# david-macmahon/BLDistributedDataProducts.jl

Measured on AMD Instinct MI355X. Metric: filterbank GB/s reduced (node) + % HBM roofline, 8-bank 0000 band, higher is better.
Workload: dtype f32

## Files before the change

bldistributeddataproducts.jl_amd/csrc/bslz4.hip:

```cpp
#include <algorithm>
#include <cstring>
#include <vector>

#include "bldp_impl.h"

namespace {

inline uint32_t be32(const uint8_t *p) {
  return (uint32_t)p[0] << 24 | (uint32_t)p[1] << 16 | (uint32_t)p[2] << 8 | p[3];
}
inline uint64_t be64(const uint8_t *p) { return (uint64_t)be32(p) << 32 | be32(p + 4); }

__host__ __device__ inline uint64_t transpose8(uint64_t x) {
  uint64_t t;
  t = (x ^ (x >> 7)) & 0x00AA00AA00AA00AAull;
  x = x ^ t ^ (t << 7);
  t = (x ^ (x >> 14)) & 0x0000CCCC0000CCCCull;
  x = x ^ t ^ (t << 14);
  t = (x ^ (x >> 28)) & 0x00000000F0F0F0F0ull;
  x = x ^ t ^ (t << 28);
  return x;
}

int64_t lz4_block_host(const uint8_t *src, size_t slen, uint8_t *dst, size_t dcap) {
  size_t ip = 0, op = 0;
  while (ip < slen) {
    const uint8_t token = src[ip++];
    size_t lit = token >> 4;
    if (lit == 15) {
      uint8_t b;
      do {
        if (ip >= slen) return -1;
        b = src[ip++];
        lit += b;
      } while (b == 255);
    }
    if (ip + lit > slen || op + lit > dcap) return -1;
    memcpy(dst + op, src + ip, lit);
    ip += lit;
    op += lit;
    if (ip >= slen) break;
    if (ip + 2 > slen) return -1;
    const size_t off = (size_t)src[ip] | (size_t)src[ip + 1] << 8;
    ip += 2;
    size_t ml = token & 15;
    if (ml == 15) {
      uint8_t b;
      do {
        if (ip >= slen) return -1;
        b = src[ip++];
        ml += b;
      } while (b == 255);
    }
    ml += 4;
    if (off == 0 || off > op || op + ml > dcap) return -1;
    for (size_t i = 0; i < ml; ++i) dst[op + i] = dst[op - off + i];
    op += ml;
  }
  return (int64_t)op;
}

void bitunshuffle_host(const uint8_t *planes, uint8_t *out, size_t n, size_t es) {
  const size_t rowb = n / 8;
  for (size_t g = 0; g < rowb; ++g)
    for (size_t j = 0; j < es; ++j) {
      uint64_t x = 0;
      for (int k = 0; k < 8; ++k) x |= (uint64_t)planes[(j * 8 + k) * rowb + g] << (8 * k);
      x = transpose8(x);
      for (int t = 0; t < 8; ++t) out[(8 * g + t) * es + j] = (uint8_t)(x >> (8 * t));
    }
}

struct Task {
  uint64_t src;
  uint64_t dst;
  uint32_t clen;
  uint32_t nelem;
};
constexpr uint32_t RAW = 0xFFFFFFFFu;

struct ChunkDesc {
  uint64_t src, len, dst;
  uint64_t n, block;
  uint32_t nfull, last, tail;
  uint32_t task0;
};

int describe_chunk(const uint8_t *c, uint64_t len, uint64_t src, uint64_t dst, int es,
                   ChunkDesc *d) {
  if (len < 12) return bldp::set_error(BLDP_EINVAL, "bslz4: chunk shorter than its header");
  const uint64_t nb = be64(c);
  const uint32_t bb = be32(c + 8);
  if (nb % es || bb % es || bb == 0 || (bb / es) % 8 || bb > (1u << 24))
    return bldp::set_error(BLDP_EINVAL, "bslz4: bad header (bytes %llu, block %u, elem %d)",
                           (unsigned long long)nb, bb, es);
  d->src = src;
  d->len = len;
  d->dst = dst;
  d->n = nb / es;
  d->block = bb / es;
  d->nfull = (uint32_t)(d->n / d->block);
  uint64_t last = d->n % d->block;
  d->last = (uint32_t)(last - last % 8);
  d->tail = (uint32_t)(d->n - (uint64_t)d->nfull * d->block - d->last);
  return BLDP_OK;
}

inline uint32_t ntasks(const ChunkDesc &d) {
  return d.nfull + (d.last ? 1 : 0) + (d.tail ? 1 : 0);
}

__host__ __device__ inline uint32_t lz4_bound(uint32_t n) { return n + n / 255 + 16; }

__device__ inline uint32_t be32_dev(const uint8_t *p) {
  return (uint32_t)p[0] << 24 | (uint32_t)p[1] << 16 | (uint32_t)p[2] << 8 | p[3];
}

__global__ __launch_bounds__(64) void k_bslz4_plan(const uint8_t *__restrict__ comp,
                                                   const ChunkDesc *__restrict__ chunks,
                                                   int nchunk, int es, uint32_t cap,
                                                   Task *__restrict__ tasks, int *err) {
  const int k = blockIdx.x * 64 + threadIdx.x;
  if (k >= nchunk) return;
  const ChunkDesc d = chunks[k];
  uint64_t pos = d.src + 12, e = 0;
  const uint64_t end = d.src + d.len;
  const uint32_t nblk = d.nfull + (d.last ? 1 : 0);
  for (uint32_t b = 0; b < nblk; ++b) {
    const uint32_t ne = b < d.nfull ? (uint32_t)d.block : d.last;
    if (pos + 4 > end) { atomicOr(err, 2); return; }
    const uint32_t cl = be32_dev(comp + pos);
    if (cl > cap || pos + 4 + cl > end) { atomicOr(err, 2); return; }
    tasks[d.task0 + b] = Task{pos + 4, d.dst + e * es, cl, ne};
    pos += 4 + cl;
    e += ne;
  }
  if (pos + (uint64_t)d.tail * es != end) { atomicOr(err, 4); return; }
  if (d.tail) tasks[d.task0 + nblk] = Task{pos, d.dst + e * es, RAW, d.tail};
}

int plan_chunk(const uint8_t *c, uint64_t len, uint64_t src0, uint64_t dst0, int es,
               std::vector<Task> &tasks, uint64_t *out_bytes, uint32_t *max_block) {
  if (len < 12) return bldp::set_error(BLDP_EINVAL, "bslz4: chunk shorter than its header");
  const uint64_t nb = be64(c);
  const uint32_t bb = be32(c + 8);
  if (nb % es || bb % es || bb == 0 || (bb / es) % 8)
    return bldp::set_error(BLDP_EINVAL, "bslz4: bad header (bytes %llu, block %u, elem %d)",
                           (unsigned long long)nb, bb, es);
  const uint64_t n = nb / es, block = bb / es;
  uint64_t pos = 12, e = 0;
  const uint64_t nfull = n / block;
  uint64_t last = n % block;
  last -= last % 8;
  for (uint64_t k = 0; k < nfull + (last ? 1 : 0); ++k) {
    const uint64_t ne = k < nfull ? block : last;
    if (pos + 4 > len) return bldp::set_error(BLDP_EINVAL, "bslz4: truncated block header");
    const uint32_t cl = be32(c + pos);
    if (cl == RAW || pos + 4 + cl > len)
      return bldp::set_error(BLDP_EINVAL, "bslz4: block %llu overruns the chunk",
                             (unsigned long long)k);
    tasks.push_back(Task{src0 + pos + 4, dst0 + e * es, cl, (uint32_t)ne});
    *max_block = std::max<uint32_t>(*max_block, std::max<uint32_t>(cl, (uint32_t)(ne * es)));
    pos += 4 + cl;
    e += ne;
  }
  const uint64_t tail = n - e;
  if (pos + tail * es != len)
    return bldp::set_error(BLDP_EINVAL, "bslz4: %llu trailing bytes, expected %llu",
                           (unsigned long long)(len - pos), (unsigned long long)(tail * es));
  if (tail) tasks.push_back(Task{src0 + pos, dst0 + e * es, RAW, (uint32_t)tail});
  *out_bytes = nb;
  return BLDP_OK;
}

__global__ __launch_bounds__(64) void k_bslz4(const uint8_t *__restrict__ comp,
                                              const Task *__restrict__ tasks, int ntask,
                                              uint8_t *__restrict__ out, int es, uint32_t cap,
                                              int *err) {
  extern __shared__ uint8_t lds[];
  const int lane = threadIdx.x;
  if (*err & 6) return;
  const Task t = tasks[blockIdx.x];
  if (t.clen == RAW) {
    for (uint32_t i = lane; i < t.nelem * (uint32_t)es; i += 64) out[t.dst + i] = comp[t.src + i];
    return;
  }
  uint8_t *in = lds, *dec = lds + cap;
  const uint32_t clen = t.clen, nbytes = t.nelem * (uint32_t)es;
  if (clen > cap) {
    if (lane == 0) atomicOr(err, 1);
    return;
  }
  for (uint32_t i = lane; i < clen; i += 64) in[i] = comp[t.src + i];
  __syncthreads();
  uint32_t ip = 0, op = 0;
  bool bad = false;
  while (ip < clen) {
    const uint32_t token = in[ip++];
    uint32_t lit = token >> 4;
    if (lit == 15) {
      uint32_t b;
      do {
        if (ip >= clen) { bad = true; break; }
        b = in[ip++];
        lit += b;
      } while (b == 255);
      if (bad) break;
    }
    if (ip + lit > clen || op + lit > nbytes) { bad = true; break; }
    for (uint32_t i = lane; i < lit; i += 64) dec[op + i] = in[ip + i];
    ip += lit;
    op += lit;
    if (ip >= clen) break;
    if (ip + 2 > clen) { bad = true; break; }
    const uint32_t off = (uint32_t)in[ip] | (uint32_t)in[ip + 1] << 8;
    ip += 2;
    uint32_t ml = token & 15;
    if (ml == 15) {
      uint32_t b;
      do {
        if (ip >= clen) { bad = true; break; }
        b = in[ip++];
        ml += b;
      } while (b == 255);
      if (bad) break;
    }
    ml += 4;
    if (off == 0 || off > op || op + ml > nbytes) { bad = true; break; }
    __syncthreads();
    const uint32_t step = off < 64 ? off : 64;
    for (uint32_t r = 0; r < ml; r += step) {
      const uint32_t i = r + lane;
      if (lane < step && i < ml) dec[op + i] = dec[op - off + i];
      __syncthreads();
    }
    op += ml;
  }
  if (bad || op != nbytes) {
    if (lane == 0) atomicOr(err, 1);
    return;
  }
  __syncthreads();
  const uint32_t rowb = t.nelem / 8;
  if (es == 4) {
    for (uint32_t g = lane; g < rowb; g += 64) {
      uint32_t w[8] = {0, 0, 0, 0, 0, 0, 0, 0};
#pragma unroll
      for (int j = 0; j < 4; ++j) {
        uint64_t x = 0;
#pragma unroll
        for (int k = 0; k < 8; ++k) x |= (uint64_t)dec[(j * 8 + k) * rowb + g] << (8 * k);
        x = transpose8(x);
#pragma unroll
        for (int q = 0; q < 8; ++q) w[q] |= (uint32_t)((x >> (8 * q)) & 0xFF) << (8 * j);
      }
      uint32_t *o = reinterpret_cast<uint32_t *>(out + t.dst) + 8 * g;
#pragma unroll
      for (int q = 0; q < 8; ++q) o[q] = w[q];
    }
  } else {
    for (uint32_t g = lane; g < rowb; g += 64)
      for (int j = 0; j < es; ++j) {
        uint64_t x = 0;
        for (int k = 0; k < 8; ++k) x |= (uint64_t)dec[(j * 8 + k) * rowb + g] << (8 * k);
        x = transpose8(x);
        for (int q = 0; q < 8; ++q) out[t.dst + (8 * g + q) * es + j] = (uint8_t)(x >> (8 * q));
      }
  }
}

}

extern "C" {

BLDP_API int bldp_bslz4_info(const void *chunk, size_t nbytes, uint64_t *uncompressed_bytes,
                             uint32_t *block_bytes) {
  if (!chunk || nbytes < 12 || !uncompressed_bytes || !block_bytes)
    return bldp::set_error(BLDP_EINVAL, "bslz4: null pointer or short chunk");
  *uncompressed_bytes = be64((const uint8_t *)chunk);
  *block_bytes = be32((const uint8_t *)chunk + 8);
  return BLDP_OK;
}

BLDP_API int bldp_bslz4_decode_host(const void *chunk, size_t nbytes, int elem_size, void *out,
                                    size_t out_bytes) {
  if (!chunk || (!out && out_bytes) || elem_size <= 0)
    return bldp::set_error(BLDP_EINVAL, "bslz4: bad argument");
  std::vector<Task> tasks;
  uint64_t total = 0;
  uint32_t maxb = 0;
  int rc = plan_chunk((const uint8_t *)chunk, nbytes, 0, 0, elem_size, tasks, &total, &maxb);
  if (rc) return rc;
  if (total != out_bytes)
    return bldp::set_error(BLDP_EINVAL, "bslz4: chunk holds %llu bytes, output has %zu",
                           (unsigned long long)total, out_bytes);
  const uint8_t *c = (const uint8_t *)chunk;
  uint8_t *o = (uint8_t *)out;
  std::vector<uint8_t> dec(maxb);
  for (const Task &t : tasks) {
    const size_t nb = (size_t)t.nelem * elem_size;
    if (t.clen == RAW) {
      memcpy(o + t.dst, c + t.src, nb);
      continue;
    }
    if (lz4_block_host(c + t.src, t.clen, dec.data(), nb) != (int64_t)nb)
      return bldp::set_error(BLDP_EINVAL, "bslz4: corrupt LZ4 block at byte %llu",
                             (unsigned long long)t.src);
    bitunshuffle_host(dec.data(), o + t.dst, t.nelem, elem_size);
  }
  return BLDP_OK;
}

static int decode_launch(int nchunk, const uint8_t *comp_host, const uint8_t *comp_dev,
                         const uint64_t *chunk_off, const uint64_t *chunk_len, int elem_size,
                         uint8_t *out_dev, const uint64_t *out_off, const uint64_t *out_len,
                         int *derr_user, hipStream_t s, int **derr_used,
                         bldp::ScratchLease &lease, uint64_t host_base = 0) {
  if (nchunk < 0 || (nchunk && (!comp_host || !comp_dev || !chunk_off || !chunk_len ||
                                !out_dev || !out_off || !out_len)) ||
      elem_size <= 0 || elem_size > 64)
    return bldp::set_error(BLDP_EINVAL, "bslz4: bad argument");
  if (elem_size == 4 && ((uintptr_t)out_dev & 3))
    return bldp::set_error(BLDP_EINVAL, "bslz4: output must be 4-byte aligned");
  std::vector<ChunkDesc> descs(nchunk);
  uint64_t ntask = 0;
  uint32_t maxbb = 0;
  for (int k = 0; k < nchunk; ++k) {
    if (chunk_off[k] < host_base)
      return bldp::set_error(BLDP_EINVAL, "bslz4: chunk %d below the host staging base", k);
    int rc = describe_chunk(comp_host + (chunk_off[k] - host_base), chunk_len[k], chunk_off[k],
                            out_off[k],
                            elem_size, &descs[k]);
    if (rc) return rc;
    if (descs[k].n * (uint64_t)elem_size != out_len[k])
      return bldp::set_error(BLDP_EINVAL,
                             "bslz4: chunk %d decodes to %llu bytes, its output slot holds %llu",
                             k, (unsigned long long)(descs[k].n * elem_size),
                             (unsigned long long)out_len[k]);
    if (elem_size == 4 && (out_off[k] & 3))
      return bldp::set_error(BLDP_EINVAL, "bslz4: output offsets must be 4-byte aligned");
    descs[k].task0 = (uint32_t)ntask;
    ntask += ntasks(descs[k]);
    if (ntask > INT32_MAX) return bldp::set_error(BLDP_EINVAL, "bslz4: too many blocks");
    maxbb = std::max<uint32_t>(maxbb, (uint32_t)(descs[k].block * elem_size));
  }
  *derr_used = nullptr;
  if (ntask == 0) return BLDP_OK;
  const uint32_t cap = (lz4_bound(maxbb) + 15) & ~15u;
  if ((size_t)cap + (((size_t)maxbb + 15) & ~(size_t)15) > 64 * 1024)
    return bldp::set_error(BLDP_EINVAL, "bslz4: block of %u bytes exceeds the LDS plan", maxbb);
  const size_t dbytes = ((descs.size() * sizeof(ChunkDesc)) + 255) & ~(size_t)255;
  const size_t tbytes = ((ntask * sizeof(Task)) + 255) & ~(size_t)255;
  int rc = bldp::scratch_lease(s, dbytes + tbytes + 256, &lease);
  if (rc) return rc;
  void *ws = lease.ptr;
  ChunkDesc *ddesc = (ChunkDesc *)ws;
  Task *dtask = (Task *)((char *)ws + dbytes);
  int *derr = derr_user ? derr_user : (int *)((char *)ws + dbytes + tbytes);
  if (hipMemcpyAsync(ddesc, descs.data(), descs.size() * sizeof(ChunkDesc),
                     hipMemcpyHostToDevice, s) != hipSuccess ||
      (!derr_user && hipMemsetAsync(derr, 0, sizeof(int), s) != hipSuccess))
    return bldp::set_error(BLDP_EHIP, "bslz4: descriptor upload failed");
  hipLaunchKernelGGL(k_bslz4_plan, dim3((unsigned)((nchunk + 63) / 64)), dim3(64), 0, s,
                     comp_dev, ddesc, nchunk, elem_size, cap, dtask, derr);
  const uint32_t dcap = (maxbb + 15) & ~15u;
  hipLaunchKernelGGL(k_bslz4, dim3((unsigned)ntask), dim3(64), cap + dcap, s, comp_dev, dtask,
                     (int)ntask, out_dev, elem_size, cap, derr);
  hipError_t e = hipGetLastError();
  if (e != hipSuccess) return bldp::set_error(BLDP_EHIP, "bslz4 launch: %s", hipGetErrorString(e));
  *derr_used = derr;
  return BLDP_OK;
}

static int decode_error(int herr) {
  if (herr & 6) return bldp::set_error(BLDP_EINVAL, "bslz4: block table overruns a chunk");
  if (herr) return bldp::set_error(BLDP_EINVAL, "bslz4: corrupt LZ4 block on the device");
  return BLDP_OK;
}

BLDP_API int bldp_bslz4_decode_dev(int nchunk, const uint8_t *comp_host, const uint8_t *comp_dev,
                                   const uint64_t *chunk_off, const uint64_t *chunk_len,
                                   int elem_size, uint8_t *out_dev, const uint64_t *out_off,
                                   const uint64_t *out_len, void *stream) {
  hipStream_t s = (hipStream_t)stream;
  int *derr = nullptr;
  bldp::ScratchLease lease;
  int rc = decode_launch(nchunk, comp_host, comp_dev, chunk_off, chunk_len, elem_size, out_dev,
                         out_off, out_len, nullptr, s, &derr, lease);
  if (rc || !derr) return rc;
  int herr = 0;
  if (hipMemcpyAsync(&herr, derr, sizeof(int), hipMemcpyDeviceToHost, s) != hipSuccess ||
      hipStreamSynchronize(s) != hipSuccess)
    return bldp::set_error(BLDP_EHIP, "bslz4: synchronize failed");
  return decode_error(herr);
}

BLDP_API int bldp_bslz4_decode_dev_async(int nchunk, const uint8_t *comp_host,
                                         const uint8_t *comp_dev, const uint64_t *chunk_off,
                                         const uint64_t *chunk_len, int elem_size,
                                         uint8_t *out_dev, const uint64_t *out_off,
                                         const uint64_t *out_len, int *err_dev, void *stream) {
  if (!err_dev) return bldp::set_error(BLDP_EINVAL, "bslz4: null error word");
  int *derr = nullptr;
  bldp::ScratchLease lease;
  return decode_launch(nchunk, comp_host, comp_dev, chunk_off, chunk_len, elem_size, out_dev,
                       out_off, out_len, err_dev, (hipStream_t)stream, &derr, lease);
}

BLDP_API int bldp_bslz4_error(const int *err_dev, void *stream) {
  if (!err_dev) return bldp::set_error(BLDP_EINVAL, "bslz4: null error word");
  int herr = 0;
  hipStream_t s = (hipStream_t)stream;
  if (hipMemcpyAsync(&herr, err_dev, sizeof(int), hipMemcpyDeviceToHost, s) != hipSuccess ||
      hipStreamSynchronize(s) != hipSuccess)
    return bldp::set_error(BLDP_EHIP, "bslz4: synchronize failed");
  return decode_error(herr);
}

}

int bldp::bslz4_decode_async_at(int nchunk, const uint8_t *comp_host, uint64_t host_base,
                                const uint8_t *comp_dev, const uint64_t *chunk_off,
                                const uint64_t *chunk_len, int elem_size, uint8_t *out_dev,
                                const uint64_t *out_off, const uint64_t *out_len, int *err_dev,
                                hipStream_t s) {
  if (!err_dev) return bldp::set_error(BLDP_EINVAL, "bslz4: null error word");
  int *derr = nullptr;
  bldp::ScratchLease lease;
  return decode_launch(nchunk, comp_host, comp_dev, chunk_off, chunk_len, elem_size, out_dev,
                       out_off, out_len, err_dev, s, &derr, lease, host_base);
}
```

Before: 7418.

## Vectorize bslz4 decode: 16-byte staging, wide LDS copies, periodic match fill, 32x32 transpose

```diff
diff --git a/bldistributeddataproducts.jl_amd/csrc/bslz4.hip b/bldistributeddataproducts.jl_amd/csrc/bslz4.hip
--- a/bldistributeddataproducts.jl_amd/csrc/bslz4.hip
+++ b/bldistributeddataproducts.jl_amd/csrc/bslz4.hip
@@ -173,54 +173,194 @@
   return BLDP_OK;
 }
 
+
+__device__ inline uint32_t lds_load4(const uint8_t *lds, uint32_t s) {
+  const uint32_t *w = reinterpret_cast<const uint32_t *>(lds) + (s >> 2);
+  const uint32_t sh = s & 3;
+  const uint32_t lo = w[0];
+  const uint32_t hi = sh ? w[1] : 0;
+  return __builtin_amdgcn_alignbyte(hi, lo, sh);
+}
+
+__device__ inline uint64_t lds_peek8(const uint8_t *lds, uint32_t s) {
+  const uint64_t *q = reinterpret_cast<const uint64_t *>(lds) + (s >> 3);
+  const uint64_t lo = q[0], hi = q[1];
+  const uint32_t sh = 8 * (s & 7);
+  const uint64_t v = sh ? (lo >> sh) | (hi << (64 - sh)) : lo;
+  const uint32_t v0 = __builtin_amdgcn_readfirstlane((uint32_t)v);
+  const uint32_t v1 = __builtin_amdgcn_readfirstlane((uint32_t)(v >> 32));
+  return (uint64_t)v0 | (uint64_t)v1 << 32;
+}
+
+__device__ inline uint32_t umod24(uint32_t i, uint32_t m) {
+  const uint32_t q = (uint32_t)((float)i * __frcp_rn((float)m));
+  int32_t r = (int32_t)(i - q * m);
+  if (r < 0) r += (int32_t)m;
+  if (r >= (int32_t)m) r -= (int32_t)m;
+  return (uint32_t)r;
+}
+
+__device__ inline void lds_copy(uint8_t *lds, uint32_t dst, uint32_t src, uint32_t n, uint32_t lane) {
+  if (n <= 64) {
+    if (lane < n) lds[dst + lane] = lds[src + lane];
+    return;
+  }
+  const uint32_t h = (0u - dst) & 3, head = h < n ? h : n;
+  const uint32_t nd = (n - head) >> 2, tail0 = head + 4 * nd;
+  if (lane < head) lds[dst + lane] = lds[src + lane];
+  if (lane >= 60 && tail0 + (lane - 60) < n) lds[dst + tail0 + (lane - 60)] = lds[src + tail0 + (lane - 60)];
+  uint32_t *wd = reinterpret_cast<uint32_t *>(lds + dst + head);
+  for (uint32_t j = lane; j < nd; j += 64) wd[j] = lds_load4(lds, src + head + 4 * j);
+}
+
+__device__ inline void lds_fill_periodic(uint8_t *lds, uint32_t dst, uint32_t off, uint32_t n,
+                                         uint32_t lane) {
+  const uint8_t *p = lds + (dst - off);
+  if (n <= 64) {
+    if (lane < n) lds[dst + lane] = p[umod24(lane, off)];
+    return;
+  }
+  const uint32_t h = (0u - dst) & 3, head = h < n ? h : n;
+  const uint32_t nd = (n - head) >> 2, tail0 = head + 4 * nd;
+  if (lane < head) {
+    uint32_t r = lane;
+    if (r >= off) r -= off;
+    if (r >= off) r -= off;
+    lds[dst + lane] = p[r];
+  }
+  if (lane >= 60 && tail0 + (lane - 60) < n) {
+    uint32_t r = umod24(tail0, off) + (lane - 60);
+    if (r >= off) r -= off;
+    if (r >= off) r -= off;
+    lds[dst + tail0 + (lane - 60)] = p[r];
+  }
+  if (nd == 0) return;
+  auto gather = [&](uint32_t r) {
+    uint32_t v = p[r];
+    r = r + 1 == off ? 0 : r + 1;
+    v |= (uint32_t)p[r] << 8;
+    r = r + 1 == off ? 0 : r + 1;
+    v |= (uint32_t)p[r] << 16;
+    r = r + 1 == off ? 0 : r + 1;
+    return v | (uint32_t)p[r] << 24;
+  };
+  uint32_t *wd = reinterpret_cast<uint32_t *>(lds + dst + head);
+  if (off == 1 || off == 2 || off == 4) {
+    const uint32_t v = gather(head & (off - 1));
+    for (uint32_t j = lane; j < nd; j += 64) wd[j] = v;
+    return;
+  }
+  uint32_t r = umod24(head + 4 * lane, off);
+  const uint32_t step = umod24(256, off);
+  for (uint32_t j = lane; j < nd; j += 64) {
+    wd[j] = gather(r);
+    r += step;
+    if (r >= off) r -= off;
+  }
+}
+
+template <int J, uint32_t M>
+__device__ inline void transpose32_stage(uint32_t (&w)[32]) {
+#pragma unroll
+  for (int k = 0; k < 32; ++k)
+    if (!(k & J)) {
+      const uint32_t t = ((w[k] >> J) ^ w[k + J]) & M;
+      w[k] ^= t << J;
+      w[k + J] ^= t;
+    }
+}
+__device__ inline void transpose32(uint32_t (&w)[32]) {
+  transpose32_stage<16, 0x0000FFFFu>(w);
+  transpose32_stage<8, 0x00FF00FFu>(w);
+  transpose32_stage<4, 0x0F0F0F0Fu>(w);
+  transpose32_stage<2, 0x33333333u>(w);
+  transpose32_stage<1, 0x55555555u>(w);
+}
+
+typedef uint32_t u32x4_a4 __attribute__((ext_vector_type(4), aligned(4)));
+
 __global__ __launch_bounds__(64) void k_bslz4(const uint8_t *__restrict__ comp,
                                               const Task *__restrict__ tasks, int ntask,
                                               uint8_t *__restrict__ out, int es, uint32_t cap,
                                               int *err) {
-  extern __shared__ uint8_t lds[];
-  const int lane = threadIdx.x;
+  extern __shared__ __attribute__((aligned(16))) uint8_t lds[];
+  const uint32_t lane = threadIdx.x;
   if (*err & 6) return;
   const Task t = tasks[blockIdx.x];
   if (t.clen == RAW) {
     for (uint32_t i = lane; i < t.nelem * (uint32_t)es; i += 64) out[t.dst + i] = comp[t.src + i];
     return;
   }
-  uint8_t *in = lds, *dec = lds + cap;
   const uint32_t clen = t.clen, nbytes = t.nelem * (uint32_t)es;
   if (clen > cap) {
     if (lane == 0) atomicOr(err, 1);
     return;
   }
-  for (uint32_t i = lane; i < clen; i += 64) in[i] = comp[t.src + i];
+  const uint8_t *g = comp + t.src;
+  const uint32_t bias = (uint32_t)(reinterpret_cast<uintptr_t>(g) & 15);
+  const uint32_t in0 = bias, dec0 = cap + 16;
+  {
+    const uint32_t h = (16 - bias) & 15, head = h < clen ? h : clen;
+    const uint32_t ngran = (clen - head) >> 4, tail0 = head + 16 * ngran;
+    if (lane < head) lds[in0 + lane] = g[lane];
+    if (lane >= 48 && tail0 + (lane - 48) < clen) lds[in0 + tail0 + (lane - 48)] = g[tail0 + (lane - 48)];
+    const uint4 *gs = reinterpret_cast<const uint4 *>(g + head);
+    uint4 *ls = reinterpret_cast<uint4 *>(lds + in0 + head);
+    for (uint32_t k0 = 0; k0 < ngran; k0 += 8 * 64) {
+      uint4 v[8];
+#pragma unroll
+      for (int u = 0; u < 8; ++u) {
+        const uint32_t k = k0 + 64 * u + lane;
+        v[u] = gs[k < ngran ? k : ngran - 1];
+      }
+#pragma unroll
+      for (int u = 0; u < 8; ++u)
+        asm volatile("" : "+v"(v[u].x), "+v"(v[u].y), "+v"(v[u].z), "+v"(v[u].w));
+#pragma unroll
+      for (int u = 0; u < 8; ++u) {
+        const uint32_t k = k0 + 64 * u + lane;
+        if (k < ngran) ls[k] = v[u];
+      }
+    }
+  }
   __syncthreads();
   uint32_t ip = 0, op = 0;
+  uint64_t win = 0;
+  uint32_t wpos = 0xFFFF0000u;
+  auto byte_at = [&](uint32_t p) -> uint32_t {
+    if (p - wpos >= 8) {
+      wpos = p;
+      win = lds_peek8(lds, in0 + p);
+    }
+    return (uint32_t)(win >> (8 * (p - wpos))) & 0xFF;
+  };
   bool bad = false;
   while (ip < clen) {
-    const uint32_t token = in[ip++];
+    const uint32_t token = byte_at(ip++);
     uint32_t lit = token >> 4;
     if (lit == 15) {
       uint32_t b;
       do {
         if (ip >= clen) { bad = true; break; }
-        b = in[ip++];
+        b = byte_at(ip++);
         lit += b;
       } while (b == 255);
       if (bad) break;
     }
     if (ip + lit > clen || op + lit > nbytes) { bad = true; break; }
-    for (uint32_t i = lane; i < lit; i += 64) dec[op + i] = in[ip + i];
+    lds_copy(lds, dec0 + op, in0 + ip, lit, lane);
     ip += lit;
     op += lit;
     if (ip >= clen) break;
     if (ip + 2 > clen) { bad = true; break; }
-    const uint32_t off = (uint32_t)in[ip] | (uint32_t)in[ip + 1] << 8;
+    const uint32_t off = byte_at(ip) | byte_at(ip + 1) << 8;
     ip += 2;
     uint32_t ml = token & 15;
     if (ml == 15) {
       uint32_t b;
       do {
         if (ip >= clen) { bad = true; break; }
-        b = in[ip++];
+        b = byte_at(ip++);
         ml += b;
       } while (b == 255);
       if (bad) break;
@@ -228,12 +368,10 @@
     ml += 4;
     if (off == 0 || off > op || op + ml > nbytes) { bad = true; break; }
     __syncthreads();
-    const uint32_t step = off < 64 ? off : 64;
-    for (uint32_t r = 0; r < ml; r += step) {
-      const uint32_t i = r + lane;
-      if (lane < step && i < ml) dec[op + i] = dec[op - off + i];
-      __syncthreads();
-    }
+    if (off >= ml)
+      lds_copy(lds, dec0 + op, dec0 + op - off, ml, lane);
+    else
+      lds_fill_periodic(lds, dec0 + op, off, ml, lane);
     op += ml;
   }
   if (bad || op != nbytes) {
@@ -241,8 +379,22 @@
     return;
   }
   __syncthreads();
+  const uint8_t *dec = lds + dec0;
   const uint32_t rowb = t.nelem / 8;
-  if (es == 4) {
+  if (es == 4 && t.nelem % 32 == 0) {
+    for (uint32_t c = lane; c < rowb / 4; c += 64) {
+      uint32_t w[32];
+#pragma unroll
+      for (int r = 0; r < 32; ++r) w[r] = *reinterpret_cast<const uint32_t *>(dec + r * rowb + 4 * c);
+      transpose32(w);
+      u32x4_a4 *o = reinterpret_cast<u32x4_a4 *>(out + t.dst) + 8 * c;
+#pragma unroll
+      for (int q = 0; q < 8; ++q) {
+        u32x4_a4 v = {w[4 * q], w[4 * q + 1], w[4 * q + 2], w[4 * q + 3]};
+        o[q] = v;
+      }
+    }
+  } else if (es == 4) {
     for (uint32_t g = lane; g < rowb; g += 64) {
       uint32_t w[8] = {0, 0, 0, 0, 0, 0, 0, 0};
 #pragma unroll
@@ -347,7 +499,7 @@
   *derr_used = nullptr;
   if (ntask == 0) return BLDP_OK;
   const uint32_t cap = (lz4_bound(maxbb) + 15) & ~15u;
-  if ((size_t)cap + (((size_t)maxbb + 15) & ~(size_t)15) > 64 * 1024)
+  if ((size_t)cap + 16 + (((size_t)maxbb + 15) & ~(size_t)15) > 64 * 1024)
     return bldp::set_error(BLDP_EINVAL, "bslz4: block of %u bytes exceeds the LDS plan", maxbb);
   const size_t dbytes = ((descs.size() * sizeof(ChunkDesc)) + 255) & ~(size_t)255;
   const size_t tbytes = ((ntask * sizeof(Task)) + 255) & ~(size_t)255;
@@ -364,7 +516,7 @@
   hipLaunchKernelGGL(k_bslz4_plan, dim3((unsigned)((nchunk + 63) / 64)), dim3(64), 0, s,
                      comp_dev, ddesc, nchunk, elem_size, cap, dtask, derr);
   const uint32_t dcap = (maxbb + 15) & ~15u;
-  hipLaunchKernelGGL(k_bslz4, dim3((unsigned)ntask), dim3(64), cap + dcap, s, comp_dev, dtask,
+  hipLaunchKernelGGL(k_bslz4, dim3((unsigned)ntask), dim3(64), cap + 16 + dcap, s, comp_dev, dtask,
                      (int)ntask, out_dev, elem_size, cap, derr);
   hipError_t e = hipGetLastError();
   if (e != hipSuccess) return bldp::set_error(BLDP_EHIP, "bslz4 launch: %s", hipGetErrorString(e));
```

Result: no change. 7415 (-0.0%).
